# thowell/DirectTrajectoryOptimization.jl

Hardware: AMD Instinct MI355X
Metric: SQP iterations/sec + Jacobian nnz/sec, acrobot T=1000, 1->8 GPU (higher is better)
Workload: dtype f64

## Files before the change

directtrajectoryoptimization.jl_amd/capi.py:

```python
from __future__ import annotations

import ctypes as C
import os

from .build import LIB, build_runtime

c_double_p = C.POINTER(C.c_double)
c_int64_p = C.POINTER(C.c_int64)
c_int32_p = C.POINTER(C.c_int32)

DTO_ABI_VERSION = 4
DTO_OK = 0
STATUS_NAMES = {0: "DTO_OK", 1: "DTO_ERR_INVALID", 2: "DTO_ERR_PLUGIN", 3: "DTO_ERR_DEVICE",
                4: "DTO_ERR_UNSUPPORTED", 5: "DTO_ERR_NOT_CONVERGED"}

(IDX_STATE, IDX_ACTION, IDX_STATE_ACTION, IDX_STATE_ACTION_NEXT, IDX_DYNAMICS_CONSTRAINT,
 IDX_DYNAMICS_JACOBIAN, IDX_DYNAMICS_HESSIAN, IDX_STAGE_CONSTRAINT, IDX_STAGE_JACOBIAN,
 IDX_STAGE_HESSIAN, IDX_OBJECTIVE_HESSIAN) = range(11)


class ProblemSpec(C.Structure):
    _fields_ = [
        ("abi_version", C.c_int),
        ("model_library", C.c_char_p),
# ... 115 lines not shown
        "dto_kkt_solve_multi": [vp, C.c_int64, vp, C.c_int64, vp, C.c_int64, vp, C.c_int64, vp, C.c_int64, vp],
        "dto_kkt_multiply": [vp, vp, C.c_int64, vp, C.c_int64, vp, C.c_int64, vp, C.c_int64, vp],
        "dto_kkt_solve_refined": [vp, C.c_int, vp, C.c_int64, vp, C.c_int64, vp, C.c_int64, vp, C.c_int64, vp, vp],
        "dto_kkt_border_factor": [vp, C.c_int64, vp, C.c_int64, vp, C.c_int64, vp, C.c_int64, c_int32_p, c_int32_p, vp],
        "dto_kkt_border_solve": [vp, vp, C.c_int64, vp, C.c_int64, vp, C.c_int64, vp, C.c_int64, vp, C.c_int64, vp, C.c_int64, vp],
        "dto_kkt_border_multiply": [vp, vp, C.c_int64, vp, C.c_int64, vp, C.c_int64, vp, C.c_int64, vp, C.c_int64, vp, C.c_int64, vp],
        "dto_kkt_border_solve_refined": [vp, C.c_int, vp, C.c_int64, vp, C.c_int64, vp, C.c_int64, vp, C.c_int64, vp, C.c_int64, vp,
                                         C.c_int64, vp, vp],
        "dto_shard_range": [C.c_int64, C.c_int, C.c_int, c_int64_p, c_int64_p],
        "dto_solver_iterate": [vp, C.c_int, vp],
        "dto_solver_stats": [vp, c_int32_p, c_int32_p, c_double_p, c_double_p, c_double_p, c_double_p, c_double_p, c_double_p],
        "dto_solver_end": [vp, vp, C.c_int64, vp, C.c_int64, vp],
        "dto_solver_scalar": [vp, C.c_int, c_double_p],
        "dto_solver_peek": [vp, C.c_int, vp, C.c_int64, vp],
        "dto_solver_hessian_mode": [vp, C.POINTER(C.c_int)],
        "dto_solver_trace": [vp, C.c_int],
        "dto_solver_trace_read": [vp, c_int32_p, c_int32_p, c_double_p, c_double_p, C.c_int64, c_int64_p],
        "dto_solver_launch_op": [vp, C.c_int, vp],
        "dto_solver_footprint": [vp, c_int64_p, c_int64_p, c_int64_p, C.POINTER(C.c_int)],
        "dto_solver_set_partitions": [vp, C.c_int],
        "dto_solver_partitions": [vp, C.POINTER(C.c_int)],
        "dto_solver_fused_update": [vp, C.POINTER(C.c_int)],
        "dto_solver_set_engine": [vp, C.c_int],
        "dto_solver_engine": [vp, C.POINTER(C.c_int)],
        "dto_solver_release": [vp],
        "dto_solver_shift": [vp, C.c_int, vp],
        "dto_solver_shift_keep_rows": [vp, c_int32_p, C.c_int64],
        "dto_solver_set_bounds": [vp, C.c_int64, vp, C.c_int64, vp, C.c_int64, vp],
        "dto_solve": [vp, C.POINTER(COptions), c_double_p, c_double_p, c_double_p, c_int32_p, c_int32_p],
        "dto_device_alloc": [C.POINTER(vp), C.c_int64],
# ... 22 lines not shown
```

directtrajectoryoptimization.jl_amd/csrc/dto_kkt_kernels.hpp:

```cpp
#pragma once

#include <hip/hip_runtime.h>
#include <math.h>

#include "dto_eval_kernels.hpp"
#include "dto_model_plugin.h"

#ifndef DTO_QN_HOT
#define DTO_QN_HOT 1
#endif

#ifdef DTO_NO_NEWTON_ONLY
#define DTO_NEWTON(o) false
#else
#define DTO_NEWTON(o) ((o).newton_only != 0)
#endif

enum dto_kkt_op {
  DTO_KKT_PACK = 0,
  DTO_KKT_UNPACK = 1,
  DTO_KKT_INIT = 2,
  DTO_KKT_EVAL = 3,
  DTO_KKT_CONV = 4,
  DTO_KKT_FACTOR_SOLVE = 5,
// ... 110 lines not shown
  double* csum; double* sfac; double* xsep; double* cacc;
  long long* prof;
  double* cpart;
  const double* sigx; const double* sigc;
  const double* rhs_x; int64_t ld_rhs_x; const double* rhs_c; int64_t ld_rhs_c;
  const int* inst_of_slot;
  int fwd_rounds;
  int fwd_group;
  int* csync;
  int sb;
  int sep_cr;
  double* qn;
  const double* qn_main;
  int qn_mode, qn_col;
  const double* aos_in; double* aos_out; int64_t ld_aos; int aos_which;
  dto_solver_opts opt;
  double* refq; double* refvz; double* refvl;
};

namespace dto {

__host__ __device__ constexpr int tri(int i, int j) { return i * (i + 1) / 2 + j; }

__device__ __forceinline__ double* soa(double* base, int64_t tile, int64_t n, int64_t i) {
  return base + ((tile * n + i) << 6) + threadIdx.x;
}
__device__ __forceinline__ const double* soa(const double* base, int64_t tile, int64_t n, int64_t i) {
  return base + ((tile * n + i) << 6) + threadIdx.x;
}

// ... 168 lines not shown
  __device__ __forceinline__ SlotBufs(const dto_kkt_args& a, int64_t g0, int ntiles) {
    z.bind(a.z, g0, a.Nz, ntiles); lam.bind(a.lam, g0, a.Nc, ntiles); zl.bind(a.zl, g0, a.Nz, ntiles); zu.bind(a.zu, g0, a.Nz, ntiles);
    s.bind(a.s, g0, a.Ni, ntiles); zs.bind(a.zs, g0, a.Ni, ntiles); dz.bind(a.dz, g0, a.Nz, ntiles);
    dlam.bind(a.dlam, g0, a.Nc, ntiles); ds.bind(a.ds, g0, a.Ni, ntiles);
    rec.bind(a.rec, g0, a.rec_total, ntiles); fac.bind(a.fac, g0, a.fac_total, ntiles);
    sigx.bind(a.sigx, g0, a.Nz, ntiles); sigc.bind(a.sigc, g0, a.Nc, ntiles); wt.bind(a.wtile, g0, a.Nw, ntiles);
  }
  __device__ __forceinline__ void slot(const dto_kkt_args& a, int tig, int lane) {
    const unsigned t512 = (unsigned)tig * 512u, l8 = (unsigned)lane * 8u;
    z.vo = zl.vo = zu.vo = sigx.vo = dz.vo = t512 * (unsigned)a.Nz + l8;
    lam.vo = sigc.vo = dlam.vo = t512 * (unsigned)a.Nc + l8;
    s.vo = zs.vo = ds.vo = t512 * (unsigned)a.Ni + l8;
    wt.vo = t512 * (unsigned)a.Nw + l8;
    rec.vo = t512 * (unsigned)a.rec_total + 2u * l8;
    fac.vo = t512 * (unsigned)a.fac_total + 2u * l8;
  }
};

template <int N>
__device__ __forceinline__ void load_params(arr<N>& w, const dto_kkt_args& a, int64_t g, int t) {
  if (a.wtile) {
    const double* src = a.wtile + ((g * a.Nw + uload(a.woff, t)) << 6) + threadIdx.x;
#pragma unroll
    for (int i = 0; i < N; ++i) w[i] = src[(int64_t)i << 6];
  } else {
    const int w0 = uload(a.woff, t);
#pragma unroll
    for (int i = 0; i < N; ++i) w[i] = uload(a.params, w0 + i);
  }
}
// ... 1530 lines not shown
constexpr bool heavy_kind() {
  using D = KindDims<M, K>;
  return D::BD * (D::BD + 1) / 2 + D::BD * D::NY > 100;
}
template <class M, int K, bool SPK>
__device__ __attribute__((noinline)) void stage_forward_cold(const dto_kkt_args& a, int64_t g, int lane, int t, double mu, double dw,
                                                            double gam, bool first, bool need, Carry<M>* cy, Spike<M>* sp, int* okneg) {
  bool ok = okneg[0] != 0;
  int nneg = okneg[1];
  const bool keep_lost = okneg[2] != 0;
  stage_forward<M, K, SPK>(a.opt, SoaSlotIO<M, K>(a, g, lane, t), mu, dw, gam, first, need, *cy, *sp, ok, nneg, keep_lost);
  okneg[0] = ok ? 1 : 0;
  okneg[1] = nneg;
}

template <int SH>
__device__ __forceinline__ void retry_update_t(const dto_solver_opts& o, int Nc, double* sc, bool ok, int nneg) {
  if (nneg != Nc) ok = false;
  sc[SC_NFACT << SH] += 1.0;
  sc[SC_NNEG << SH] = (double)nneg;
  double dw = sc[SC_TRY_DW << SH], gam = sc[SC_TRY_GAM << SH];
  const double dlast = sc[SC_DELTA_LAST << SH];
  const int attempt = (int)sc[SC_ATTEMPT << SH];
  const bool done = ok || o.newton_only || attempt >= o.max_refactor;
  if (done) {
    sc[SC_NEED << SH] = 0.0;
    sc[SC_DELTA_W << SH] = dw;
    sc[SC_GAMMA << SH] = gam;
    if (dw > 0.0 && gam != 0.0) sc[SC_DELTA_LAST << SH] = dw;
    if (dw == 0.0) sc[SC_DELTA_LAST << SH] = 0.0;
    sc[SC_LS_FAIL << SH] = ok ? 0.0 : 1.0;
    sc[SC_QN_RESET << SH] = (gam == 0.0) ? 1.0 : 0.0;
    return;
  }
  if (gam != 0.0) {
    const bool skip_ladder = (sc[SC_GAMMA << SH] == 0.0) && (((int)sc[SC_ITER << SH]) % 4 != 0);
    if (dw == 0.0 && !skip_ladder) dw = (dlast == 0.0) ? o.delta_w_init : fmax(o.delta_w_min, o.kappa_w_minus * dlast);
    else if (!skip_ladder) dw *= (dlast == 0.0) ? o.kappa_w_plus_first : o.kappa_w_plus;
    if (skip_ladder || dw > o.delta_w_exact_cap) {
      gam = 0.0;
      dw = o.delta_w_init;
    }
  } else {
    dw = (dw == 0.0) ? o.delta_w_init : dw * o.kappa_w_plus;
    if (dw > o.delta_w_max) dw = o.delta_w_max;
  }
  sc[SC_TRY_DW << SH] = dw;
  sc[SC_TRY_GAM << SH] = gam;
  sc[SC_ATTEMPT << SH] = (double)(attempt + 1);
}

__device__ __forceinline__ void retry_update(const dto_kkt_args& a, double* sc, bool ok, int nneg) {
  retry_update_t<6>(a.opt, (int)a.Nc, sc, ok, nneg);
}

__device__ __forceinline__ int nth_set_bit(unsigned long long m, int n) {
  int pos = 0;
#pragma unroll
  for (int w = 32; w >= 1; w >>= 1) {
    const int c = __popcll((m >> pos) & ((1ull << w) - 1ull));
    if (n >= c) { n -= c; pos += w; }
  }
  return pos;
// ... 82 lines not shown
              }
              stage_forward<M, K, false>(a.opt, IO(a, bufs, run, t, cur), mu, dw, gam, false, need, cy, sp, ok, nneg, keep_lost);
              if (!__any(need && (ok || keep_lost))) { lost = true; break; }
            }
          };
          if (run.bounded) sweep(std::integral_constant<bool, true>{}); else sweep(std::integral_constant<bool, false>{});
        }
      });
    }
    if (need) retry_update(a, sc, ok, nneg);
    if (a.opt.newton_only) return;
    if (k > 1) __builtin_amdgcn_fence(__ATOMIC_SEQ_CST, "workgroup");
  }
}

template <class M, bool CHUNKED>
__device__ __forceinline__ void kkt_fwd_body(const dto_kkt_args& a) {
  if constexpr (!CHUNKED) {
    kkt_fwd_seq_body<M>(a);
  } else {
  const int64_t g = blockIdx.x / a.P;
  const int p = blockIdx.x % a.P;
  double* sc = a.scal + ((g * SC_COUNT) << 6) + threadIdx.x;
  {
    const bool need = sc[SC_STATUS << 6] == 0.0 && sc[SC_NEED << 6] != 0.0;
    if (!__any(need)) return;
    const double mu = sc[SC_MU << 6];
    const double dw = sc[SC_TRY_DW << 6] + (DTO_QN_HOT && a.opt.qn_lbfgs ? sc[SC_QN_SIGMA << 6] : 0.0), gam = sc[SC_TRY_GAM << 6];
    const int t0 = uload(a.cstart, p), t1 = uload(a.cstart, p + 1);
    Carry<M> cy;
// ... 83 lines not shown
}

template <class M>
__global__ __launch_bounds__(WAVE) void k_kkt_fwd(dto_kkt_args a) { kkt_fwd_body<M, true>(a); }
template <class M>
__global__ __launch_bounds__(WAVE, DTO_SEQ_FWD_OCC) void k_kkt_fwd_seq(dto_kkt_args a) {
  if (a.fwd_started && threadIdx.x == 0) atomicAdd(a.fwd_started, 1);
  kkt_fwd_body<M, false>(a);
  if (a.tile_fwd_tag) {
    __builtin_amdgcn_fence(__ATOMIC_RELEASE, "agent");
    const int k = a.fwd_group > 1 ? a.fwd_group : 1, g0 = (int)blockIdx.x * k;
    if ((int)threadIdx.x < k && g0 + (int)threadIdx.x < a.G)
      __hip_atomic_store(a.tile_fwd_tag + g0 + threadIdx.x, a.sweep_tag, __ATOMIC_RELAXED, __HIP_MEMORY_SCOPE_AGENT);
  }
}

#ifndef DTO_SEP_CR_MAX_INST
#define DTO_SEP_CR_MAX_INST 4
#endif
__device__ __forceinline__ void sep_lds_fence() {
  __builtin_amdgcn_fence(__ATOMIC_ACQ_REL, "wavefront");
  __builtin_amdgcn_wave_barrier();
}
template <class M>
__device__ __forceinline__ void kkt_sep_cr(const dto_kkt_args& a, const int64_t g, const int li, bool& ok_out, int& nneg_out) {
  using CS = ChunkSum<M>;
  constexpr int N = CS::N, NT = CS::NT, NN = N * N;
  __shared__ double sh_lo[64 * NN], sh_f[64 * NN], sh_g[64 * NN], sh_y[64 * N], sh_x[64 * N];
  const dto_solver_opts& o = a.opt;
  const int j = threadIdx.x;
// ... 611 lines not shown
#ifndef DTO_FUSE_SWEEPS
#define DTO_FUSE_SWEEPS 0
#endif
#if DTO_FUSE_SWEEPS
template <class M>
__global__ __launch_bounds__(WAVE, 1) void k_kkt_fwdbwd_seq(dto_kkt_args a) {
  kkt_fwd_body<M, false>(a);
  __builtin_amdgcn_fence(__ATOMIC_SEQ_CST, "agent");
  kkt_bwd_body<M, false>(a);
}
#endif
__host__ __device__ inline int fwd_seq_blocks(const dto_kkt_args& a) {
  const int k = a.fwd_group > 1 ? a.fwd_group : 1;
  return (a.G + k - 1) / k;
}
static __global__ __launch_bounds__(WAVE) void k_kkt_bwd_gate(dto_kkt_args a) {
  for (int spin = 0; spin < 100000; ++spin) {
    if (__hip_atomic_load(a.fwd_started, __ATOMIC_RELAXED, __HIP_MEMORY_SCOPE_AGENT) >= fwd_seq_blocks(a)) return;
    __builtin_amdgcn_s_sleep(127);
  }
}
template <class M>
__global__ __launch_bounds__(WAVE, DTO_SEQ_BWD_OCC) void k_kkt_bwd_early(dto_kkt_args a) {
  if (a.tile_bwd_tag[blockIdx.x] == a.sweep_tag) return;
  if (__hip_atomic_load(a.tile_fwd_tag + blockIdx.x, __ATOMIC_RELAXED, __HIP_MEMORY_SCOPE_AGENT) != a.sweep_tag) return;
  __builtin_amdgcn_fence(__ATOMIC_ACQUIRE, "agent");
  kkt_bwd_body<M, false>(a);
  if (threadIdx.x == 0) a.tile_bwd_tag[blockIdx.x] = a.sweep_tag;
}
template <class M>
// ... 1056 lines not shown
            hipLaunchKernelGGL(k_kkt_fwd<M>, dim3(gp), dim3(WAVE), 0, st, a);
            if (sep_wide) hipLaunchKernelGGL(k_kkt_sep_cr<M>, dim3((unsigned)a.G * 64u), dim3(WAVE), 0, st, a);
            else hipLaunchKernelGGL(k_kkt_sep<M>, dim3((unsigned)a.G), dim3(WAVE), 0, st, a);
          }
          if (a.csync) {
            hipLaunchKernelGGL(k_kkt_bwd_post<M>, dim3(gp), dim3(WAVE), 0, st, a);
            break;
          }
          hipLaunchKernelGGL(k_kkt_bwd<M>, dim3(gp), dim3(WAVE), 0, st, a);
        } else {
          const int per = a.fwd_rounds > 0 ? a.fwd_rounds : rounds;
#if DTO_FUSE_SWEEPS
          if (per == rounds) { hipLaunchKernelGGL(k_kkt_fwdbwd_seq<M>, dim3(gp), dim3(WAVE), 0, st, a); } else
#endif
          {
          for (int r = 0; r < rounds; r += per) hipLaunchKernelGGL(k_kkt_fwd_seq<M>, dim3((unsigned)fwd_seq_blocks(a)), dim3(WAVE), 0, st, a);
          hipLaunchKernelGGL(k_kkt_bwd_seq<M>, dim3(gp), dim3(WAVE), 0, st, a);
          }
        }
        hipLaunchKernelGGL(k_kkt_post, dim3((unsigned)a.G), dim3(WAVE), 0, st, a);
        break;
      }
      case DTO_KKT_FWD:
        if (a.P > 1) hipLaunchKernelGGL(k_kkt_fwd<M>, dim3((unsigned)((int64_t)a.G * a.P)), dim3(WAVE), 0, st, a);
        else hipLaunchKernelGGL(k_kkt_fwd_seq<M>, dim3((unsigned)fwd_seq_blocks(a)), dim3(WAVE), 0, st, a);
        break;
      case DTO_KKT_SEP: hipLaunchKernelGGL(k_kkt_sep<M>, dim3((unsigned)a.G), dim3(WAVE), 0, st, a); break;
      case DTO_KKT_BWD:
        if (a.P > 1) hipLaunchKernelGGL(k_kkt_bwd<M>, dim3((unsigned)((int64_t)a.G * a.P)), dim3(WAVE), 0, st, a);
        else hipLaunchKernelGGL(k_kkt_bwd_seq<M>, dim3((unsigned)((int64_t)a.G * a.P)), dim3(WAVE), 0, st, a);
        break;
      case DTO_KKT_BWD_GATE:
        if (!a.fwd_started) return (int)hipErrorInvalidValue;
        hipLaunchKernelGGL(k_kkt_bwd_gate, dim3(1), dim3(WAVE), 0, st, a);
        break;
      case DTO_KKT_BWD_EARLY:
      case DTO_KKT_BWD_REST:
        if (a.P != 1 || !a.tile_fwd_tag || !a.tile_bwd_tag) return (int)hipErrorInvalidValue;
        if (op == DTO_KKT_BWD_EARLY) hipLaunchKernelGGL(k_kkt_bwd_early<M>, dim3((unsigned)a.G), dim3(WAVE), 0, st, a);
// ... 54 lines not shown
```

directtrajectoryoptimization.jl_amd/csrc/dto_solver.cpp:

```cpp
#include <hip/hip_runtime.h>

#include <algorithm>
#include <chrono>
#include <cmath>
#include <cstdio>
#include <cstdint>
#include <cstdlib>
#include <cstring>
#include <vector>

#include "../../include/dto.h"
#include "dto_kkt_kernels.hpp"
#include "dto_point_rules.hpp"
#include "dto_im_kernels.hpp"
#include "dto_wide_kernels.hpp"
#include "dto_border_kernels.hpp"
#include "dto_problem.hpp"
#include "dto_host_globalization.hpp"

#define HIP_TRY(expr)                                       \
  do {                                                      \
    hipError_t e_ = (expr);                                 \
    if (e_ != hipSuccess) return dto::hip_fail(e_, #expr);  \
  } while (0)
// ... 5 lines not shown
  DevBuf<double> wtile;
  DevBuf<int> d_inst_of_slot, d_src_slot;
  DevBuf<double> repack_tmp;
  DevBuf<double> sigx, sigc;
  DevBuf<int> d_ioff;
  DevBuf<int64_t> d_recoff, d_facoff;
  DevBuf<dto_stage_run> d_runs;
  DevBuf<double> d_lo, d_hi;
  DevBuf<double> z, lam, zl, zu, s, zs;
  DevBuf<int> tile_fwd_tag, tile_bwd_tag, fwd_started;
  DevBuf<double> qn;
  DevBuf<double> refq, refvz, refvl, rec_bak;
  DevBuf<double> z_alt, lam_alt;
  DevBuf<double> dz, dlam, ds;
  DevBuf<double> rec, fac, part, lspart, scal, filt;
  DevBuf<double> csum, sfac, xsep, cacc, cpart;
  DevBuf<int> csync;
  DevBuf<int> d_cstart_all;
};

struct SolverState : SolverBufs {
  int64_t B = 0;
  int G = 0;
  int64_t Ni = 0, rec_total = 0, fac_total = 0, n_bnd = 0;
  bool use_wtile = false;
  int G_active = 0;
  std::vector<int> inst_of_slot, slot_of_inst;
  bool use_sigx = false, use_sigc = false, assembled = false;
  std::vector<int> ioff;
  std::vector<int64_t> recoff, facoff;
  int n_runs = 0;
  int sweep_tag = 0;
  hipStream_t stream_lo = nullptr;
  hipEvent_t ev_fork = nullptr, ev_join = nullptr;
  SolverState* cols = nullptr;
  int fuse_state = 0;
  int sb = 8;
  int P = 1;
  int P0 = 1;
  int P_cap = 1;
  int forced_P = 0;
  int n_simd = 1024;
  std::vector<int> cstart;
  int* d_cstart = nullptr;
  dto_kkt_info info{};
  dto_solver_opts opt{};
  dto_options user{};
  bool begun = false;
  std::vector<double> h_scal;

  void release() {
    static_cast<SolverBufs&>(*this) = SolverBufs();
    d_cstart = nullptr; n_runs = 0; fuse_state = 0; sweep_tag = 0;
    if (stream_lo) { (void)hipStreamDestroy(stream_lo); stream_lo = nullptr; }
    if (ev_fork) { (void)hipEventDestroy(ev_fork); ev_fork = nullptr; }
    if (ev_join) { (void)hipEventDestroy(ev_join); ev_join = nullptr; }
    use_wtile = false;
    use_sigx = use_sigc = assembled = false;
    G_active = 0;
    inst_of_slot.clear(); slot_of_inst.clear();
    B = 0; G = 0;
    delete cols; cols = nullptr;
  }
  ~SolverState() { release(); }
};
template <class S>
struct ReleaseOnError {
  S* s;
// ... 37 lines not shown
  o.tol = u.tol; o.s_max = u.s_max; o.dual_inf_tol = u.dual_inf_tol; o.constr_viol_tol = u.constr_viol_tol;
  o.compl_inf_tol = u.compl_inf_tol; o.max_iter = u.max_iter;
  o.acceptable_tol = u.acceptable_tol; o.acceptable_iter = u.acceptable_iter; o.acceptable_dual_inf_tol = u.acceptable_dual_inf_tol;
  o.acceptable_constr_viol_tol = u.acceptable_constr_viol_tol; o.acceptable_compl_inf_tol = u.acceptable_compl_inf_tol;
  o.acceptable_obj_change_tol = u.acceptable_obj_change_tol;
  o.diverging_iterates_tol = u.diverging_iterates_tol; o.mu_target = u.mu_target;
  o.mu_init = u.mu_init; o.kappa_eps = 10.0; o.kappa_mu = 0.2; o.theta_mu = 1.5; o.tau_min = 0.99;
  o.bound_push = 1e-2; o.bound_frac = 1e-2;
  o.delta_c = u.delta_c; o.delta_w_init = u.delta_w_init; o.delta_w_min = 1e-20; o.delta_w_max = 1e20;
  if (const char* e = getenv("DTO_DW_FLOOR")) { const double v = atof(e); if (v > 0.0) o.delta_w_min = v; }
  o.kappa_w_minus = 1.0 / 3.0; o.kappa_w_plus = 8.0; o.kappa_w_plus_first = 100.0;
  o.delta_w_exact_cap = 100.0;
  if (const char* e = getenv("DTO_EXACT_CAP")) o.delta_w_exact_cap = atof(e);
  o.eta_armijo = 1e-4; o.rho_penalty = 0.1; o.piv_tol = 1e-9;
  o.max_refactor = 9;
  o.watchdog_trigger = 2; o.watchdog_trials = 4;
  if (const char* e = getenv("DTO_WATCHDOG")) sscanf(e, "%d,%d", &o.watchdog_trigger, &o.watchdog_trials);
  o.newton_only = 0; o.fixed_delta_w = 0.0;
  o.warm = 0; o.mu_warm = 0.0;
  o.ls_penalty = u.line_search == DTO_LS_PENALTY_FILTER ? 1 : 0; o.ls_switch = u.penalty_switch_theta;
  if (const char* e = getenv("DTO_LS_MERIT")) o.ls_penalty = atoi(e);
  o.pen_gn = 1;
  o.qn_lbfgs = u.hessian_approximation == DTO_HESSIAN_LBFGS ? 1 : 0;
  o.cost_hess_scale = o.qn_lbfgs ? 0.0 : 1.0;
  if (const char* e = getenv("DTO_PEN_GN")) o.pen_gn = atoi(e);
}

struct BorderStats;

static int bordered_step(Problem* p, const dto_batch* b, const double* mu, int64_t ldmu, const double* dw, double delta_c,
// ... 1132 lines not shown
}

#ifndef DTO_FWD_GROUP_MAX
#define DTO_FWD_GROUP_MAX 4
#endif
static int fwd_group_for(Problem* p, const dto_kkt_args& a) {
  const SolverState& S = *p->solver;
  if (a.P != 1 || a.fwd_rounds > 0 || a.opt.newton_only || a.G < 2) return 1;
  int k = (int)std::min<int64_t>(DTO_FWD_GROUP_MAX, (int64_t)a.G / std::max(1, S.n_simd));
  if (const char* e = getenv("DTO_FWD_GROUP")) { const int v = atoi(e); if (v >= 1) k = std::min(v, 64); }
  const int64_t rows = std::max<int64_t>({a.Nz, a.Nc, a.Ni, a.Nw, a.rec_total, a.fac_total, 1});
  k = (int)std::min<int64_t>(k, (((int64_t)1 << 31) - 1) / (rows * 512));
  return std::max(1, std::min(k, a.G));
}

static int kkt_launch(Problem* p, int op, const dto_kkt_args& a, hipStream_t st) {
  if ((op == DTO_KKT_FWD || op == DTO_KKT_FACTOR_SOLVE || op == DTO_KKT_BWD_GATE) && a.fwd_group == 0 && p->solver) {
    const int k = fwd_group_for(p, a);
    if (k > 1) {
      dto_kkt_args b = a;
      b.fwd_group = k;
      return kkt_launch(p, op, b, st);
    }
  }
  LaunchTrace* tr = (p->trace && p->trace->on && p->trace->recs.size() < LaunchTrace::MAX_RECS) ? p->trace : nullptr;
  int e0 = -1, e1 = -1;
  if (tr) {
    e0 = tr->take(); e1 = tr->take();
    if (e0 < 0 || e1 < 0) tr = nullptr;
    else HIP_TRY(hipEventRecord(tr->pool[(size_t)e0], st));
  }
  const int rc = p->vt->launch_kkt(op, &a, (void*)st);
  if (rc != 0) return hip_fail((hipError_t)rc, "KKT kernel launch");
  if (tr) {
    HIP_TRY(hipEventRecord(tr->pool[(size_t)e1], st));
    tr->recs.push_back({op, tr->iteration, e0, e1});
  }
// ... 1761 lines not shown
      if ((rc = dto::kkt_launch(p, DTO_KKT_FACTOR_SOLVE, a, st))) return rc;
      a.qn_mode = 2;
      if ((rc = dto::kkt_launch(p, DTO_KKT_QN_RHS, a, st))) return rc;
      a.qn_mode = 0; a.qn_col = 0;
    }
    if ((rc = dto::kkt_launch(p, DTO_KKT_LINESEARCH, a, st))) return rc;
    if ((rc = dto::kkt_launch(p, DTO_KKT_LS_REDUCE, a, st))) return rc;
    if (qn && (rc = dto::kkt_launch(p, DTO_KKT_QN_SAVE, a, st))) return rc;
    if (!(it + 1 < n && it + 1 <= n_fused))
      if ((rc = dto::kkt_launch(p, DTO_KKT_UPDATE, a, st))) return rc;
  }
  if (p->trace && p->trace->on) ++p->trace->iteration;
  return DTO_OK;
}

int dto_solver_hessian_mode(dto_problem* h, int* mode) {
  Problem* p = reinterpret_cast<Problem*>(h);
  if (!p || !mode) return set_error(DTO_ERR_INVALID, "null argument");
  *mode = p->hessian_mode_last;
  return DTO_OK;
}

int dto_solver_trace(dto_problem* h, int on) {
  Problem* p = reinterpret_cast<Problem*>(h);
  if (!p) return set_error(DTO_ERR_INVALID, "null argument");
  if (p->vt->launch_wide) return set_error(DTO_ERR_UNSUPPORTED, "dto_solver_trace: the tile path has no launch trace");
  if (!p->trace) p->trace = new dto::LaunchTrace();
  if (on) p->trace->clear();
  p->trace->on = on != 0;
  return DTO_OK;
// ... 1072 lines not shown
```

directtrajectoryoptimization.jl_amd/solver.py:

```python
from __future__ import annotations

import ctypes as C
from dataclasses import dataclass
from typing import List, Optional, Sequence

import numpy as np

from . import capi
from .model import Bound, Constraint, Cost, Dynamics, GeneralConstraint
from .plugin import Structure, build_plugin


@dataclass
class Options:
    tol: float = 1e-6
    s_max: float = 100.0
    max_iter: int = 1000
    max_cpu_time: float = 300.0
    dual_inf_tol: float = 1.0
    constr_viol_tol: float = 1.0e-3
    compl_inf_tol: float = 1.0e-3
    acceptable_tol: float = 1.0e-6
    acceptable_iter: int = 15
    acceptable_dual_inf_tol: float = 1.0e10
# ... 945 lines not shown
    def trace(self, on: bool = True):
        capi.check(self._solve_nlp._lib.dto_solver_trace(self._solve_nlp._h, 1 if on else 0))

    def read_trace(self):
        n = C.c_int64(0)
        capi.check(self._solve_nlp._lib.dto_solver_trace_read(self._solve_nlp._h, None, None, None, None, 0, C.byref(n)))
        cnt = int(n.value)
        op, it = np.zeros(max(cnt, 1), np.int32), np.zeros(max(cnt, 1), np.int32)
        t0, dt = np.zeros(max(cnt, 1)), np.zeros(max(cnt, 1))
        capi.check(self._solve_nlp._lib.dto_solver_trace_read(self._solve_nlp._h, op.ctypes.data_as(capi.c_int32_p), it.ctypes.data_as(capi.c_int32_p),
                                                       capi.dptr(t0), capi.dptr(dt), cnt, C.byref(n)))
        names = {v: k for k, v in self.KKT_OPS.items()}
        names.update({16: "kkt_bwd_early", 17: "kkt_bwd_rest", 18: "kkt_bwd_gate", 25: "kkt_refine"})
        return dict(op=op[:cnt], name=[names.get(int(o), str(int(o))) for o in op[:cnt]], iteration=it[:cnt], start_ms=t0[:cnt], duration_ms=dt[:cnt])

    def hessian_mode_last(self) -> str:
        v = C.c_int(-1)
        capi.check(self._solve_nlp._lib.dto_solver_hessian_mode(self._solve_nlp._h, C.byref(v)))
        return {-1: "none", 0: "exact", 1: "lbfgs", 2: "sr1"}[v.value]

    def scalar_batch(self, name: str):
        out = np.zeros(self._B)
        capi.check(self._solve_nlp._lib.dto_solver_scalar(self._solve_nlp._h, capi.SCALARS.index(name), capi.dptr(out)))
        return out

    PEEK = dict(z=0, multipliers=1, dz=2, dmultipliers=3, z_lower=5, z_upper=6, slack=7, slack_multipliers=8, dslack=9)

    def peek_batch(self, name: str):
        import torch
        which = self.PEEK[name]
# ... 445 lines not shown
```

include/dto.h:

```cpp
#ifndef DTO_H
#define DTO_H

#include <stdint.h>

#ifdef __cplusplus
extern "C" {
#endif

#define DTO_ABI_VERSION 4

enum dto_status {
  DTO_OK = 0,
  DTO_ERR_INVALID = 1,
  DTO_ERR_PLUGIN = 2,
  DTO_ERR_DEVICE = 3,
  DTO_ERR_UNSUPPORTED = 4,
  DTO_ERR_NOT_CONVERGED = 5
};

#define DTO_FEATURE_GRAD 1
#define DTO_FEATURE_JAC 2
#define DTO_FEATURE_HESS 4

typedef struct dto_problem dto_problem;
// ... 177 lines not shown
int dto_solver_stats(dto_problem* p, int32_t* status, int32_t* iterations, double* objective, double* constr_viol,
                     double* dual_inf, double* mu, double* delta_w, double* alpha);
int dto_solver_launch_op(dto_problem* p, int op, void* stream);
int dto_solver_set_partitions(dto_problem* p, int partitions);
int dto_solver_partitions(dto_problem* p, int* partitions);
int dto_solver_fused_update(dto_problem* p, int* fused);
int dto_solver_set_engine(dto_problem* p, int engine);
int dto_solver_release(dto_problem* p);
int dto_solver_engine(dto_problem* p, int* engine);
int dto_solver_footprint(dto_problem* p, int64_t* record_doubles, int64_t* factor_doubles, int64_t* num_slacks,
                         int* factor_rounds );
int dto_solver_scalar(dto_problem* p, int slot, double* out);
int dto_solver_peek(dto_problem* p, int which, double* out, int64_t ld, void* stream);
int dto_solver_end(dto_problem* p, double* x_out, int64_t ldxo, double* mu_out, int64_t ldmuo, void* stream);
int dto_solver_hessian_mode(dto_problem* p, int* mode);
int dto_solver_trace(dto_problem* p, int on);
int dto_solver_trace_read(dto_problem* p, int32_t* op, int32_t* iteration, double* start_ms, double* duration_ms, int64_t capacity,
                          int64_t* count);

int dto_solve(dto_problem* p, const dto_options* opt, const double* x0, double* x, double* mu, int32_t* status,
              int32_t* iterations);

int dto_device_alloc(void** ptr, int64_t bytes);
int dto_device_free(void* ptr);
int dto_copy_to_device(void* dst, const void* src, int64_t bytes);
int dto_copy_to_host(void* dst, const void* src, int64_t bytes);
int dto_device_synchronize(void);
int dto_device_count(int* n);
int dto_shard_range(int64_t total, int rank, int world, int64_t* first, int64_t* count);

// ... 5 lines not shown
```

Measured before the change: 3.089 million.

## Speculatively factor the next inertia-correction rung in idle lanes during forward sweep

Adds a forward-sweep kernel variant where, on retry passes, idle wavefront lanes factor the next regularization rung (the next delta_w/gamma from the ladder) into a spare factor buffer, alongside the lanes retrying the current rung. If the current attempt fails but the speculative one succeeds, its factor is copied back and one refactor pass is skipped. The spare buffer is either the unused second half of the factor storage or a newly allocated one. It is enabled only under narrow conditions (single partition, no quasi-Newton, low occupancy) and adds copy traffic, extra memory, and more complex lane mapping.

```diff
diff --git a/directtrajectoryoptimization.jl_amd/capi.py b/directtrajectoryoptimization.jl_amd/capi.py
--- a/directtrajectoryoptimization.jl_amd/capi.py
+++ b/directtrajectoryoptimization.jl_amd/capi.py
@@ -153,6 +153,7 @@
         "dto_solver_scalar": [vp, C.c_int, c_double_p],
         "dto_solver_peek": [vp, C.c_int, vp, C.c_int64, vp],
         "dto_solver_hessian_mode": [vp, C.POINTER(C.c_int)],
+        "dto_solver_forward_ahead": [vp, C.POINTER(C.c_int)],
         "dto_solver_trace": [vp, C.c_int],
         "dto_solver_trace_read": [vp, c_int32_p, c_int32_p, c_double_p, c_double_p, C.c_int64, c_int64_p],
         "dto_solver_launch_op": [vp, C.c_int, vp],
diff --git a/directtrajectoryoptimization.jl_amd/csrc/dto_kkt_kernels.hpp b/directtrajectoryoptimization.jl_amd/csrc/dto_kkt_kernels.hpp
--- a/directtrajectoryoptimization.jl_amd/csrc/dto_kkt_kernels.hpp
+++ b/directtrajectoryoptimization.jl_amd/csrc/dto_kkt_kernels.hpp
@@ -148,6 +148,7 @@
   const double* qn_main;
   int qn_mode, qn_col;
   const double* aos_in; double* aos_out; int64_t ld_aos; int aos_which;
+  int fwd_ahead_rows;
   dto_solver_opts opt;
   double* refq; double* refvz; double* refvl;
 };
@@ -346,6 +347,57 @@
     wt.vo = t512 * (unsigned)a.Nw + l8;
     rec.vo = t512 * (unsigned)a.rec_total + 2u * l8;
     fac.vo = t512 * (unsigned)a.fac_total + 2u * l8;
+  }
+};
+
+struct AheadFacBuf {
+  __amdgpu_buffer_rsrc_t r, r2;
+  unsigned vo, vo2;
+  static constexpr unsigned OFF = 0x80000000u;
+  __device__ __forceinline__ void bind(const double* home, const double* copy, int64_t rows) {
+    r = __builtin_amdgcn_make_buffer_rsrc(const_cast<double*>(home), 0, (int)(rows * 512), 0x00020000);
+    r2 = __builtin_amdgcn_make_buffer_rsrc(const_cast<double*>(copy), 0, (int)(rows * 512), 0x00020000);
+    vo = vo2 = OFF;
+  }
+  __device__ __forceinline__ void slot(int lane, bool ahead) {
+    vo = ahead ? OFF : (unsigned)lane * 16u;
+    vo2 = ahead ? (unsigned)lane * 16u : OFF;
+  }
+  __device__ __forceinline__ void ld2(int row0, int k, double& v0, double& v1) const {
+    const dto_v4i q = __builtin_amdgcn_raw_buffer_load_b128(r, vo, (row0 << 9) + (k << 10), 0);
+    v0 = __builtin_bit_cast(double, dto_v2i{q[0], q[1]});
+    v1 = __builtin_bit_cast(double, dto_v2i{q[2], q[3]});
+  }
+  __device__ __forceinline__ double ld1p(int row0, int i) const {
+    return __builtin_bit_cast(double, __builtin_amdgcn_raw_buffer_load_b64(r, vo + (i & 1) * 8u, (row0 << 9) + ((i >> 1) << 10), 0));
+  }
+  __device__ __forceinline__ void st2(int row0, int k, double v0, double v1, bool on) const {
+    const dto_v2i a0 = __builtin_bit_cast(dto_v2i, v0), a1 = __builtin_bit_cast(dto_v2i, v1);
+    const dto_v4i q{a0[0], a0[1], a1[0], a1[1]};
+    __builtin_amdgcn_raw_buffer_store_b128(q, r, on ? vo : OFF, (row0 << 9) + (k << 10), 0);
+    __builtin_amdgcn_raw_buffer_store_b128(q, r2, on ? vo2 : OFF, (row0 << 9) + (k << 10), 0);
+  }
+  __device__ __forceinline__ void st1p(int row0, int i, double v, bool on) const {
+    const dto_v2i q = __builtin_bit_cast(dto_v2i, v);
+    __builtin_amdgcn_raw_buffer_store_b64(q, r, (on && vo != OFF) ? vo + (i & 1) * 8u : OFF, (row0 << 9) + ((i >> 1) << 10), 0);
+    __builtin_amdgcn_raw_buffer_store_b64(q, r2, (on && vo2 != OFF) ? vo2 + (i & 1) * 8u : OFF, (row0 << 9) + ((i >> 1) << 10), 0);
+  }
+};
+struct AheadBufs {
+  SlotBuf z, lam, zl, zu, s, zs, dz, dlam, ds, rec, sigx, sigc, wt;
+  AheadFacBuf fac;
+  __device__ __forceinline__ AheadBufs(const dto_kkt_args& a, int64_t g, const double* fac_home, const double* fac_copy) {
+    z.bind(a.z, g, a.Nz, 1); lam.bind(a.lam, g, a.Nc, 1); zl.bind(a.zl, g, a.Nz, 1); zu.bind(a.zu, g, a.Nz, 1);
+    s.bind(a.s, g, a.Ni, 1); zs.bind(a.zs, g, a.Ni, 1); dz.bind(a.dz, g, a.Nz, 1);
+    dlam.bind(a.dlam, g, a.Nc, 1); ds.bind(a.ds, g, a.Ni, 1);
+    rec.bind(a.rec, g, a.rec_total, 1); fac.bind(fac_home, fac_copy, a.fac_total);
+    sigx.bind(a.sigx, g, a.Nz, 1); sigc.bind(a.sigc, g, a.Nc, 1); wt.bind(a.wtile, g, a.Nw, 1);
+  }
+  __device__ __forceinline__ void slot(int lane, bool ahead) {
+    const unsigned l8 = (unsigned)lane * 8u;
+    z.vo = zl.vo = zu.vo = sigx.vo = dz.vo = lam.vo = sigc.vo = dlam.vo = s.vo = zs.vo = ds.vo = wt.vo = l8;
+    rec.vo = 2u * l8;
+    fac.slot(lane, ahead);
   }
 };
 
@@ -1906,8 +1958,29 @@
   okneg[1] = nneg;
 }
 
+struct LadderRung { double dw, gam; };
+template <class Skip>
+__host__ __device__ __forceinline__ LadderRung ladder_next(const dto_solver_opts& o, double dw, double gam, double dlast, Skip&& skip) {
+  if (gam != 0.0) {
+    const bool skip_ladder = skip();
+    if (dw == 0.0 && !skip_ladder) dw = (dlast == 0.0) ? o.delta_w_init : fmax(o.delta_w_min, o.kappa_w_minus * dlast);
+    else if (!skip_ladder) dw *= (dlast == 0.0) ? o.kappa_w_plus_first : o.kappa_w_plus;
+    if (skip_ladder || dw > o.delta_w_exact_cap) {
+      gam = 0.0;
+      dw = o.delta_w_init;
+    }
+  } else {
+    dw = (dw == 0.0) ? o.delta_w_init : dw * o.kappa_w_plus;
+    if (dw > o.delta_w_max) dw = o.delta_w_max;
+  }
+  return LadderRung{dw, gam};
+}
+__host__ __device__ __forceinline__ LadderRung ladder_next(const dto_solver_opts& o, double dw, double gam, double dlast, double sc_gamma,
+                                                           int iter) {
+  return ladder_next(o, dw, gam, dlast, [&] { return (sc_gamma == 0.0) && (iter % 4 != 0); });
+}
 template <int SH>
-__device__ __forceinline__ void retry_update_t(const dto_solver_opts& o, int Nc, double* sc, bool ok, int nneg) {
+__host__ __device__ __forceinline__ void retry_update_t(const dto_solver_opts& o, int Nc, double* sc, bool ok, int nneg) {
   if (nneg != Nc) ok = false;
   sc[SC_NFACT << SH] += 1.0;
   sc[SC_NNEG << SH] = (double)nneg;
@@ -1925,20 +1998,10 @@
     sc[SC_QN_RESET << SH] = (gam == 0.0) ? 1.0 : 0.0;
     return;
   }
-  if (gam != 0.0) {
-    const bool skip_ladder = (sc[SC_GAMMA << SH] == 0.0) && (((int)sc[SC_ITER << SH]) % 4 != 0);
-    if (dw == 0.0 && !skip_ladder) dw = (dlast == 0.0) ? o.delta_w_init : fmax(o.delta_w_min, o.kappa_w_minus * dlast);
-    else if (!skip_ladder) dw *= (dlast == 0.0) ? o.kappa_w_plus_first : o.kappa_w_plus;
-    if (skip_ladder || dw > o.delta_w_exact_cap) {
-      gam = 0.0;
-      dw = o.delta_w_init;
-    }
-  } else {
-    dw = (dw == 0.0) ? o.delta_w_init : dw * o.kappa_w_plus;
-    if (dw > o.delta_w_max) dw = o.delta_w_max;
-  }
-  sc[SC_TRY_DW << SH] = dw;
-  sc[SC_TRY_GAM << SH] = gam;
+  const LadderRung nx =
+      ladder_next(o, dw, gam, dlast, [&] { return (sc[SC_GAMMA << SH] == 0.0) && (((int)sc[SC_ITER << SH]) % 4 != 0); });
+  sc[SC_TRY_DW << SH] = nx.dw;
+  sc[SC_TRY_GAM << SH] = nx.gam;
   sc[SC_ATTEMPT << SH] = (double)(attempt + 1);
 }
 
@@ -2051,6 +2114,154 @@
   }
 }
 
+template <class M, int K>
+struct SoaSlotAheadIO : SoaSlotIO<M, K> {
+  __device__ __forceinline__ SoaSlotAheadIO(const dto_kkt_args& a_, int64_t g_, int lane_, int t_, double* fac_tile)
+      : SoaSlotIO<M, K>(a_, g_, lane_, t_) {
+    this->facp = fac_tile + (uload(a_.facoff, t_) << 6) + 2 * lane_;
+  }
+};
+template <class M, int K>
+__device__ __attribute__((noinline)) void stage_forward_cold_ahead(const dto_kkt_args& a, int64_t g, int lane, double* fac_tile, int t,
+                                                                  double mu, double dw, double gam, bool need, Carry<M>* cy,
+                                                                  Spike<M>* sp, int* okneg) {
+  bool ok = okneg[0] != 0;
+  int nneg = okneg[1];
+  const bool keep_lost = okneg[2] != 0;
+  stage_forward<M, K, false>(a.opt, SoaSlotAheadIO<M, K>(a, g, lane, t, fac_tile), mu, dw, gam, false, need, *cy, *sp, ok, nneg, keep_lost);
+  okneg[0] = ok ? 1 : 0;
+  okneg[1] = nneg;
+}
+
+template <class M>
+__device__ __forceinline__ void ahead_copy_home(const dto_kkt_args& a, double* home, const double* copy, int lane) {
+  for (int r = 0; r < a.n_runs; ++r) {
+    const dto_stage_run run = load_run(a.runs, r);
+    dispatch_uniform<M>(run.kind, [&](auto kc) {
+      constexpr int NPR = (KindDims<M, decltype(kc)::value>::F_CX + 1) / 2;
+      if constexpr (NPR > 0) {
+        const int total = (run.t1 - run.t0) * NPR;
+        auto at = [&](int i) { return ((run.fac0 + (int64_t)(i / NPR) * run.facs) << 6) + ((int64_t)(i % NPR) << 7) + 2 * lane; };
+        for (int i0 = (int)threadIdx.x; i0 < total; i0 += 8 * WAVE) {
+          double2 v[8];
+#pragma unroll
+          for (int u = 0; u < 8; ++u)
+            if (i0 + u * WAVE < total) v[u] = *reinterpret_cast<const double2*>(copy + at(i0 + u * WAVE));
+#pragma unroll
+          for (int u = 0; u < 8; ++u)
+            if (i0 + u * WAVE < total) *reinterpret_cast<double2*>(home + at(i0 + u * WAVE)) = v[u];
+        }
+      }
+    });
+  }
+}
+
+template <class M>
+__device__ __forceinline__ void kkt_fwd_seq_ahead_body(const dto_kkt_args& a) {
+  const int64_t g = blockIdx.x;
+  if (g >= a.G) return;
+  const int tid = threadIdx.x;
+  double* const fac_home = a.fac + ((g * a.fac_total) << 6);
+  double* const fac_copy = fac_home + ((int64_t)a.fwd_ahead_rows << 6);
+  AheadBufs bufs(a, g, fac_home, fac_copy);
+  double* const sc_tile = a.scal + ((g * SC_COUNT) << 6);
+  for (int pass = 0; pass <= a.opt.max_refactor; ++pass) {
+    const unsigned long long m = __ballot(sc_tile[(SC_STATUS << 6) + tid] == 0.0 && sc_tile[(SC_NEED << 6) + tid] != 0.0);
+    const int c = __popcll(m);
+    if (c == 0) return;
+    const bool ahead = pass > 0 && tid >= c;
+    bool mine = pass > 0 ? tid < 2 * c : ((m >> tid) & 1ull) != 0;
+    const int lane = (pass > 0 && mine) ? nth_set_bit(m, (ahead ? tid - c : tid) & (WAVE - 1)) : tid;
+    double* sc = sc_tile + lane;
+    int attempt = (int)sc[SC_ATTEMPT << 6];
+    double try_dw = sc[SC_TRY_DW << 6], gam = sc[SC_TRY_GAM << 6];
+    if (ahead) {
+      if (mine && attempt < a.opt.max_refactor) {
+        const LadderRung nx = ladder_next(a.opt, try_dw, gam, sc[SC_DELTA_LAST << 6], sc[SC_GAMMA << 6], (int)sc[SC_ITER << 6]);
+        try_dw = nx.dw;
+        gam = nx.gam;
+        attempt += 1;
+      } else {
+        mine = false;
+      }
+    }
+    const bool need = mine;
+    bufs.slot(lane, ahead);
+    double* const fac_tile = ahead ? fac_copy : fac_home;
+    const double mu = sc[SC_MU << 6];
+    const double dw = try_dw + (DTO_QN_HOT && a.opt.qn_lbfgs ? sc[SC_QN_SIGMA << 6] : 0.0);
+    Carry<M> cy;
+    Spike<M> sp;
+#pragma unroll
+    for (int i = 0; i < M::MAX_NX * (M::MAX_NX + 1) / 2; ++i) cy.P[i] = sp.RLL[i] = 0.0;
+#pragma unroll
+    for (int i = 0; i < M::MAX_NX; ++i) cy.py[i] = sp.rL[i] = 0.0;
+#pragma unroll
+    for (int i = 0; i < M::MAX_NX * M::MAX_NX; ++i) sp.Cx[i] = 0.0;
+    bool ok = true;
+    int nneg = 0;
+    const bool keep_lost = attempt >= a.opt.max_refactor;
+    bool lost = false;
+    for (int r = 0; r < a.n_runs && !lost; ++r) {
+      const dto_stage_run run = load_run(a.runs, r);
+      dispatch_uniform<M>(run.kind, [&](auto kc) {
+        constexpr int K = decltype(kc)::value;
+        if constexpr (heavy_kind<M, K>()) {
+          for (int t = run.t0; t < run.t1; ++t) {
+            Carry<M> cyc = cy;
+            Spike<M> spc = sp;
+            int okneg[3] = {ok ? 1 : 0, nneg, keep_lost ? 1 : 0};
+            const dto_kkt_args acold = a;
+            stage_forward_cold_ahead<M, K>(acold, g, lane, fac_tile, t, mu, dw, gam, need, &cyc, &spc, okneg);
+            cy = cyc;
+            ok = okneg[0] != 0;
+            nneg = okneg[1];
+            if (!__any(need && (ok || keep_lost))) { lost = true; break; }
+          }
+        } else {
+          auto sweep = [&](auto bounded) {
+            using IO = SoaPreIO<M, K, decltype(bounded)::value, false, false, AheadBufs>;
+            constexpr bool PRE = DTO_SEQ_PREFETCH_FWD && sizeof(typename IO::In) <= DTO_SEQ_PREFETCH_MAX * sizeof(double);
+            typename IO::In nxt, cur;
+            if (PRE) nxt.load(bufs, run, run.t0);
+            for (int t = run.t0; t < run.t1; ++t) {
+              if (PRE) {
+                cur = nxt;
+                nxt.load(bufs, run, min(t + 1, run.t1 - 1));
+              } else {
+                cur.load(bufs, run, t);
+              }
+              stage_forward<M, K, false>(a.opt, IO(a, bufs, run, t, cur), mu, dw, gam, false, need, cy, sp, ok, nneg, keep_lost);
+              if (!__any(need && (ok || keep_lost))) { lost = true; break; }
+            }
+          };
+          if (run.bounded) sweep(std::integral_constant<bool, true>{}); else sweep(std::integral_constant<bool, false>{});
+        }
+      });
+    }
+    const int partner = (tid + c) & (WAVE - 1);
+    const int p_on = __shfl(need && ahead ? 1 : 0, partner), p_ok = __shfl(ok ? 1 : 0, partner), p_nneg = __shfl(nneg, partner);
+    bool take = false;
+    if (need && !ahead) {
+      retry_update(a, sc, ok, nneg);
+      if (tid + c < WAVE && p_on != 0 && sc[SC_NEED << 6] != 0.0) {
+        retry_update(a, sc, p_ok != 0, p_nneg);
+        take = sc[SC_NEED << 6] == 0.0;
+      }
+    }
+    __builtin_amdgcn_fence(__ATOMIC_SEQ_CST, "workgroup");
+    unsigned long long tk = __ballot(take);
+    if (tk != 0) {
+      while (tk != 0) {
+        const int src = __ffsll((long long)tk) - 1;
+        tk &= tk - 1;
+        ahead_copy_home<M>(a, fac_home, fac_copy, __shfl(lane, src));
+      }
+      __builtin_amdgcn_fence(__ATOMIC_SEQ_CST, "workgroup");
+    }
+  }
+}
+
 template <class M, bool CHUNKED>
 __device__ __forceinline__ void kkt_fwd_body(const dto_kkt_args& a) {
   if constexpr (!CHUNKED) {
@@ -2164,6 +2375,10 @@
       __hip_atomic_store(a.tile_fwd_tag + g0 + threadIdx.x, a.sweep_tag, __ATOMIC_RELAXED, __HIP_MEMORY_SCOPE_AGENT);
   }
 }
+template <class M>
+__global__ __launch_bounds__(WAVE, DTO_SEQ_FWD_OCC) void k_kkt_fwd_seq_ahead(dto_kkt_args a) {
+  kkt_fwd_seq_ahead_body<M>(a);
+}
 
 #ifndef DTO_SEP_CR_MAX_INST
 #define DTO_SEP_CR_MAX_INST 4
@@ -2805,6 +3020,9 @@
   const int k = a.fwd_group > 1 ? a.fwd_group : 1;
   return (a.G + k - 1) / k;
 }
+inline bool fwd_seq_ahead(const dto_kkt_args& a) {
+  return a.fwd_ahead_rows != 0 && a.P == 1 && a.fwd_rounds <= 0 && a.fwd_group <= 1 && !a.opt.newton_only && !a.tile_fwd_tag && !a.fwd_started;
+}
 static __global__ __launch_bounds__(WAVE) void k_kkt_bwd_gate(dto_kkt_args a) {
   for (int spin = 0; spin < 100000; ++spin) {
     if (__hip_atomic_load(a.fwd_started, __ATOMIC_RELAXED, __HIP_MEMORY_SCOPE_AGENT) >= fwd_seq_blocks(a)) return;
@@ -3891,6 +4109,8 @@
           if (per == rounds) { hipLaunchKernelGGL(k_kkt_fwdbwd_seq<M>, dim3(gp), dim3(WAVE), 0, st, a); } else
 #endif
           {
+          if (fwd_seq_ahead(a)) hipLaunchKernelGGL(k_kkt_fwd_seq_ahead<M>, dim3((unsigned)a.G), dim3(WAVE), 0, st, a);
+          else
           for (int r = 0; r < rounds; r += per) hipLaunchKernelGGL(k_kkt_fwd_seq<M>, dim3((unsigned)fwd_seq_blocks(a)), dim3(WAVE), 0, st, a);
           hipLaunchKernelGGL(k_kkt_bwd_seq<M>, dim3(gp), dim3(WAVE), 0, st, a);
           }
@@ -3900,6 +4120,7 @@
       }
       case DTO_KKT_FWD:
         if (a.P > 1) hipLaunchKernelGGL(k_kkt_fwd<M>, dim3((unsigned)((int64_t)a.G * a.P)), dim3(WAVE), 0, st, a);
+        else if (fwd_seq_ahead(a)) hipLaunchKernelGGL(k_kkt_fwd_seq_ahead<M>, dim3((unsigned)a.G), dim3(WAVE), 0, st, a);
         else hipLaunchKernelGGL(k_kkt_fwd_seq<M>, dim3((unsigned)fwd_seq_blocks(a)), dim3(WAVE), 0, st, a);
         break;
       case DTO_KKT_SEP: hipLaunchKernelGGL(k_kkt_sep<M>, dim3((unsigned)a.G), dim3(WAVE), 0, st, a); break;
diff --git a/directtrajectoryoptimization.jl_amd/csrc/dto_solver.cpp b/directtrajectoryoptimization.jl_amd/csrc/dto_solver.cpp
--- a/directtrajectoryoptimization.jl_amd/csrc/dto_solver.cpp
+++ b/directtrajectoryoptimization.jl_amd/csrc/dto_solver.cpp
@@ -43,6 +43,7 @@
   DevBuf<double> z_alt, lam_alt;
   DevBuf<double> dz, dlam, ds;
   DevBuf<double> rec, fac, part, lspart, scal, filt;
+  DevBuf<double> fac_ahead;
   DevBuf<double> csum, sfac, xsep, cacc, cpart;
   DevBuf<int> csync;
   DevBuf<int> d_cstart_all;
@@ -64,6 +65,8 @@
   hipEvent_t ev_fork = nullptr, ev_join = nullptr;
   SolverState* cols = nullptr;
   int fuse_state = 0;
+  int ahead_state = 0;
+  int ahead_source = 0;
   int sb = 8;
   int P = 1;
   int P0 = 1;
@@ -80,7 +83,7 @@
 
   void release() {
     static_cast<SolverBufs&>(*this) = SolverBufs();
-    d_cstart = nullptr; n_runs = 0; fuse_state = 0; sweep_tag = 0;
+    d_cstart = nullptr; n_runs = 0; fuse_state = 0; ahead_state = 0; sweep_tag = 0;
     if (stream_lo) { (void)hipStreamDestroy(stream_lo); stream_lo = nullptr; }
     if (ev_fork) { (void)hipEventDestroy(ev_fork); ev_fork = nullptr; }
     if (ev_join) { (void)hipEventDestroy(ev_join); ev_join = nullptr; }
@@ -148,6 +151,7 @@
   if (const char* e = getenv("DTO_EXACT_CAP")) o.delta_w_exact_cap = atof(e);
   o.eta_armijo = 1e-4; o.rho_penalty = 0.1; o.piv_tol = 1e-9;
   o.max_refactor = 9;
+  if (const char* e = getenv("DTO_MAX_REFACTOR")) o.max_refactor = std::max(0, atoi(e));
   o.watchdog_trigger = 2; o.watchdog_trials = 4;
   if (const char* e = getenv("DTO_WATCHDOG")) sscanf(e, "%d,%d", &o.watchdog_trigger, &o.watchdog_trials);
   o.newton_only = 0; o.fixed_delta_w = 0.0;
@@ -1310,6 +1314,40 @@
   return std::max(1, std::min(k, a.G));
 }
 
+static int fwd_ahead_for(Problem* p, const dto_kkt_args& a) {
+  SolverState& S = *p->solver;
+  const char* e = getenv("DTO_FWD_AHEAD");
+  const int v = e ? atoi(e) : -1;
+  S.ahead_source = 0;
+  if (v == 0) return 0;
+  if (a.P != 1 || a.fwd_rounds > 0 || a.opt.newton_only || a.opt.qn_lbfgs || S.info.quasi_newton || a.opt.max_refactor < 2) return 0;
+  if (a.tile_fwd_tag || a.fwd_started || a.fac != S.fac || a.G > S.n_simd || a.G > S.G) return 0;
+  if (v < 0 && (int64_t)a.G * 4 > (int64_t)S.n_simd * 3) return 0;
+  int only = 0;
+  if (const char* so = getenv("DTO_FWD_AHEAD_SOURCE")) only = atoi(so);
+  const int64_t row_max = 0x7fffffff;
+  if (only != 2 && S.G_active > 0 && a.G == S.G_active && 2 * (int64_t)a.G <= S.G && (int64_t)a.G * S.fac_total <= row_max) {
+    S.ahead_source = 1;
+    return (int)((int64_t)a.G * S.fac_total);
+  }
+  if (only == 1 || S.G > S.n_simd) return 0;
+  if (S.ahead_state == 0) {
+    S.ahead_state = -1;
+    const size_t need = (size_t)S.G * 64 * (size_t)S.fac_total + 64;
+    size_t free_b = 0, total_b = 0;
+    if (hipMemGetInfo(&free_b, &total_b) != hipSuccess) { (void)hipGetLastError(); return 0; }
+    if (v < 0 && free_b < need * sizeof(double) + total_b / 8) return 0;
+    if (S.fac_ahead.alloc(need) != hipSuccess) { (void)hipGetLastError(); return 0; }
+    S.ahead_state = 1;
+  }
+  if (S.ahead_state < 0) return 0;
+  const uintptr_t f0 = (uintptr_t)(double*)S.fac, f1 = (uintptr_t)(double*)S.fac_ahead;
+  const int64_t rows = f1 >= f0 ? (int64_t)((f1 - f0 + 511) / 512) : -(int64_t)((f0 - f1) / 512);
+  if (rows == 0 || rows > row_max || rows < -row_max) return 0;
+  S.ahead_source = 2;
+  return (int)rows;
+}
+
 static int kkt_launch(Problem* p, int op, const dto_kkt_args& a, hipStream_t st) {
   if ((op == DTO_KKT_FWD || op == DTO_KKT_FACTOR_SOLVE || op == DTO_KKT_BWD_GATE) && a.fwd_group == 0 && p->solver) {
     const int k = fwd_group_for(p, a);
@@ -1317,6 +1355,14 @@
       dto_kkt_args b = a;
       b.fwd_group = k;
       return kkt_launch(p, op, b, st);
+    }
+    if ((op == DTO_KKT_FWD || op == DTO_KKT_FACTOR_SOLVE) && a.fwd_ahead_rows == 0) {
+      if (const int rows = fwd_ahead_for(p, a)) {
+        dto_kkt_args b = a;
+        b.fwd_group = 1;
+        b.fwd_ahead_rows = rows;
+        return kkt_launch(p, op, b, st);
+      }
     }
   }
   LaunchTrace* tr = (p->trace && p->trace->on && p->trace->recs.size() < LaunchTrace::MAX_RECS) ? p->trace : nullptr;
@@ -3108,6 +3154,13 @@
   return DTO_OK;
 }
 
+int dto_solver_forward_ahead(dto_problem* h, int* source) {
+  Problem* p = reinterpret_cast<Problem*>(h);
+  if (!p || !source) return set_error(DTO_ERR_INVALID, "null argument");
+  *source = p->solver ? p->solver->ahead_source : 0;
+  return DTO_OK;
+}
+
 int dto_solver_hessian_mode(dto_problem* h, int* mode) {
   Problem* p = reinterpret_cast<Problem*>(h);
   if (!p || !mode) return set_error(DTO_ERR_INVALID, "null argument");
diff --git a/directtrajectoryoptimization.jl_amd/solver.py b/directtrajectoryoptimization.jl_amd/solver.py
--- a/directtrajectoryoptimization.jl_amd/solver.py
+++ b/directtrajectoryoptimization.jl_amd/solver.py
@@ -983,6 +983,11 @@
         names.update({16: "kkt_bwd_early", 17: "kkt_bwd_rest", 18: "kkt_bwd_gate", 25: "kkt_refine"})
         return dict(op=op[:cnt], name=[names.get(int(o), str(int(o))) for o in op[:cnt]], iteration=it[:cnt], start_ms=t0[:cnt], duration_ms=dt[:cnt])
 
+    def forward_ahead(self) -> int:
+        v = C.c_int(0)
+        capi.check(self._solve_nlp._lib.dto_solver_forward_ahead(self._solve_nlp._h, C.byref(v)))
+        return v.value
+
     def hessian_mode_last(self) -> str:
         v = C.c_int(-1)
         capi.check(self._solve_nlp._lib.dto_solver_hessian_mode(self._solve_nlp._h, C.byref(v)))
diff --git a/include/dto.h b/include/dto.h
--- a/include/dto.h
+++ b/include/dto.h
@@ -215,6 +215,7 @@
 int dto_solver_peek(dto_problem* p, int which, double* out, int64_t ld, void* stream);
 int dto_solver_end(dto_problem* p, double* x_out, int64_t ldxo, double* mu_out, int64_t ldmuo, void* stream);
 int dto_solver_hessian_mode(dto_problem* p, int* mode);
+int dto_solver_forward_ahead(dto_problem* p, int* source);
 int dto_solver_trace(dto_problem* p, int on);
 int dto_solver_trace_read(dto_problem* p, int32_t* op, int32_t* iteration, double* start_ms, double* duration_ms, int64_t capacity,
                           int64_t* count);
```

After: 2.950 million. 0.955x the previous value.
